# artis-mcrt/artis

Hardware: AMD Instinct MI355X
Metric: packet-steps/sec (higher is better)
Workload: dtype f64

## Files before the change

### artis_amd/csrc/artis_engine.hip

```cpp
#include <hip/hip_runtime.h>
#include <rccl/rccl.h>

#include <dlfcn.h>

#include <cstdio>
#include <cstdlib>
#include <algorithm>
#include <chrono>
#include <cstring>
#include <string>
#include <type_traits>
#include <utility>
#include <vector>
#include <cmath>

#include "model_build.h"
#include "engine_config.h"
#include "physics.h"
#include "radfield_fit.h"
#include "ion_balance.h"
#include "spectra.h"

#include <rocprim/device/device_radix_sort.hpp>

// ... 821 lines not shown
        kind = NEXT_RPKT;
      } else {
        kind = kpkt_blackbody_case(env, type, cellindex) ? NEXT_BB : NEXT_KPKT;
      }
    }
  }
  append_by_kind(kind, (int32_t)i, cellindex, nu_cmf, L);
}

__global__ void __launch_bounds__(BLOCK) k_count_waiting(Env env, int32_t *counts, int32_t *other) {
  const int64_t i = (int64_t)blockIdx.x * BLOCK + threadIdx.x;
  if (i >= env.P.n) return;
  const PktHot &h = env.P.hot[i];
  const int type = h.type;
  const bool active = type_handled(type) && h.prop_time < env.S.ts_end;
  const bool waiting = h.pend != PEND_NONE || h.ma_level >= 0;
  if (!(waiting || active)) return;
  const int c = env.M.propcell_nonemptymgi[h.cellindex];
  if ((active && type_gamma(type) && !waiting) || c < 0)
    atomicAdd(other, 1);
  else
    atomicAdd(&counts[c], 1);
}
__global__ void __launch_bounds__(BLOCK) k_sort_hist(const int32_t *keys, int32_t n, int32_t *hist) {
  const int64_t i = (int64_t)blockIdx.x * BLOCK + threadIdx.x;
  if (i < n) atomicAdd(&hist[keys[i]], 1);
}
constexpr int SCAN_TILE = 8192;
__global__ void __launch_bounds__(1024) k_scan_tiles(int32_t *hist, int32_t nkeys, int32_t *tile_totals) {
  __shared__ int32_t part[1024];
  const int t = threadIdx.x;
  const int64_t base = (int64_t)blockIdx.x * SCAN_TILE + (int64_t)t * 8;
  int32_t v[8];
  int32_t sum = 0;
#pragma unroll
  for (int k = 0; k < 8; k++) {
    v[k] = (base + k < nkeys) ? hist[base + k] : 0;
    sum += v[k];
  }
  part[t] = sum;
  __syncthreads();
  for (int off = 1; off < 1024; off <<= 1) {
    const int32_t add = (t >= off) ? part[t - off] : 0;
    __syncthreads();
    part[t] += add;
    __syncthreads();
  }
  int32_t run = part[t] - sum;
#pragma unroll
// ... 9 lines not shown
  int32_t carry = 0;
  for (int start = 0; start < ntiles; start += 1024) {
    const int i = start + t;
    const int32_t v = (i < ntiles) ? tile_totals[i] : 0;
    part[t] = v;
    __syncthreads();
    for (int off = 1; off < 1024; off <<= 1) {
      const int32_t add = (t >= off) ? part[t - off] : 0;
      __syncthreads();
      part[t] += add;
      __syncthreads();
    }
    if (i < ntiles) tile_totals[i] = carry + part[t] - v;
    carry += part[1023];
    __syncthreads();
  }
}
__global__ void __launch_bounds__(1024) k_scan_add(int32_t *hist, int32_t nkeys, const int32_t *tile_totals) {
  const int32_t off = tile_totals[blockIdx.x];
  const int64_t base = (int64_t)blockIdx.x * SCAN_TILE + (int64_t)threadIdx.x * 8;
#pragma unroll
  for (int k = 0; k < 8; k++)
    if (base + k < nkeys) hist[base + k] += off;
}
__global__ void __launch_bounds__(BLOCK) k_sort_scatter(const int32_t *list, const int32_t *keys, int32_t n, int32_t *offsets, int32_t *out) {
  const int64_t i = (int64_t)blockIdx.x * BLOCK + threadIdx.x;
  if (i < n) out[atomicAdd(&offsets[keys[i]], 1)] = list[i];
}
constexpr int SORT_LDS_KEYS = 8192;
constexpr int SORT_LDS_GRID = 2048;
__global__ void __launch_bounds__(BLOCK) k_sort_hist_lds(const int32_t *keys, int32_t n, int32_t *hist, int32_t nkeys) {
  __shared__ int32_t h[SORT_LDS_KEYS];
  for (int k = threadIdx.x; k < nkeys; k += BLOCK) h[k] = 0;
  __syncthreads();
  const int64_t chunk = ((int64_t)n + gridDim.x - 1) / gridDim.x;
  const int64_t lo = chunk * blockIdx.x, hi = (lo + chunk < n) ? lo + chunk : n;
  for (int64_t i = lo + threadIdx.x; i < hi; i += BLOCK) atomicAdd(&h[keys[i]], 1);
  __syncthreads();
  for (int k = threadIdx.x; k < nkeys; k += BLOCK)
    if (h[k] != 0) atomicAdd(&hist[k], h[k]);
}
__global__ void __launch_bounds__(BLOCK) k_sort_scatter_lds(const int32_t *list, const int32_t *keys, int32_t n, int32_t *offsets, int32_t *out,
                                                            int32_t nkeys) {
  __shared__ int32_t h[SORT_LDS_KEYS];
  for (int k = threadIdx.x; k < nkeys; k += BLOCK) h[k] = 0;
  __syncthreads();
  const int64_t chunk = ((int64_t)n + gridDim.x - 1) / gridDim.x;
  const int64_t lo = chunk * blockIdx.x, hi = (lo + chunk < n) ? lo + chunk : n;
  for (int64_t i = lo + threadIdx.x; i < hi; i += BLOCK) atomicAdd(&h[keys[i]], 1);
  __syncthreads();
// ... 1139 lines not shown
  }
  __syncthreads();
  if (threadIdx.x < ARTIS_NSTATS && lstats[threadIdx.x] != 0) atomicAdd(&gstats[threadIdx.x], lstats[threadIdx.x]);
}
#endif

inline int nblocks(int64_t n) { return (int)((n + BLOCK - 1) / BLOCK); }

struct SpecState;
void spec_free(SpecState *st);
struct RfState;
void rf_free(RfState *st);
struct IbState;
void ib_free(IbState *st);

}

struct LastCall {
  double propagate_ms = 0., kms[NEXT_NKINDS] = {}, kms_tail = 0., fill_ms = 0.;
  int64_t klaunches[NEXT_NKINDS] = {}, kthreads[NEXT_NKINDS] = {}, nlaunches = 0;
  int64_t sweeps = 0, tile_fills = 0, sparse_fills = 0, cells_filled = 0, listed = 0, parked = 0;
  int64_t pool_resets = 0;
  int32_t thermal_variants = 0, est_forms = 0;
};
struct artis_amd_engine {
  int device = 0;
  EngineConfig cfg;
  double cache_budget = 0.;
  SpecState *spec = nullptr;
  RfState *rf = nullptr;
  IbState *ib = nullptr;
  bool fit_since_step = false;
  ModelOwned own;
  std::vector<void *> model_allocs;
  std::vector<void *> cell_allocs;
  std::vector<void *> cache_allocs;
  DevModel M{};
  DevModel Mh{};
  artis_model model_copy{};
  std::vector<int32_t> own_matransblock_start;
  DevCells C{};
  DevCache K{};
  DevStep S{};
  DevEst E{};
  bool have_cells = false;
  bool expopac_own = false;
// ... 21 lines not shown
  int32_t *d_target_level = nullptr;
  double *d_est = nullptr;
  int64_t est_ndoubles = 0;
  int64_t nvspec = 0, nvgrid = 0;
  unsigned long long *d_stats = nullptr;
  int32_t *d_err = nullptr;
  int32_t *h_counts = nullptr;
  int64_t npackets = -1;
  void *d_pkt = nullptr;
  void *d_pkt_snapshot = nullptr;
  size_t pkt_bytes = 0;
  PktStore P{};
  artis_packet *d_aos = nullptr;
  int64_t aos_capacity = 0;
  bool aos_valid = false;
  int32_t *d_lists[NEXT_NKINDS][2] = {};
  int32_t *d_keys[NEXT_NKINDS][2] = {};
  int32_t *d_sorted = nullptr;
  int32_t *d_perm = nullptr;
  bool use_perm = false;
  bool slot_order_by_cell = true;
  int32_t *d_hist = nullptr;
  int32_t *d_tiles = nullptr;
  int32_t *d_count = nullptr;
  int32_t *d_cursors = nullptr;
  int ncu = 256;
  double *d_gamma_ws = nullptr;
  int32_t *d_gamma_gi = nullptr;
  int32_t *d_gamma_n = nullptr;
  int64_t ws_capacity = 0;
  hipEvent_t ev0 = nullptr, ev1 = nullptr, ev2 = nullptr, ev3 = nullptr;
  LastCall last;
  int tail_max = ARTIS_OPT_DETAILED_BF_ESTIMATORS_ON ? 16384 : 4096;
  bool tail_always = false;
  int32_t *d_fill_cells = nullptr;
  bool sparse_fill = true;
  int64_t sparse_max_listed = 16384;
  bool park_tails = true;
  int64_t park_at = 3145728;
  int64_t last_pool_used = 0, last_pool_cap = 0;
  double ma_hotfrac = 1.;
  bool vpkt_cont_lds = true;
  bool tile_zigzag = false;
  bool tile_adapt = true;
  int64_t tile_block = 0;
  bool pool_keep = true;
// ... 157 lines not shown
  env.S = e->S;
  env.E = e->E;
  env.est_stride = 8;
  env.pair_stride = 2;
  env.P = e->P;
  env.stats = nullptr;
  env.gamma_ws = e->d_gamma_ws;
  env.bfev = e->bf_defer ? e->d_bfev : nullptr;
  env.bfev_count = e->d_bfev_count;
  env.bfev_cap = e->bfev_cap;
  env.bfrate_kept = (e->bf_defer && e->ntiles == 1) ? e->d_bfrate_kept : nullptr;
  env.gamma_gi = e->d_gamma_gi;
  env.gamma_n = e->d_gamma_n;
  env.errflag = e->d_err;
  env.vpkt_queue = e->d_vpkt_queue;
  env.vpkt_count = e->d_vpkt_count;
  env.vpkt_cap = e->vpkt_cap;
#ifdef ARTIS_VISIT_COUNTS
  env.visit_counts = e->d_visit_counts;
#endif
  return env;
}

void free_packet_buffers(artis_amd_engine *e) {
  void **singles[] = {&e->d_pkt, &e->d_pkt_snapshot, (void **)&e->d_sorted, (void **)&e->d_perm, (void **)&e->d_gamma_ws,
                      (void **)&e->d_gamma_gi, (void **)&e->d_gamma_n, (void **)&e->d_bfev, (void **)&e->d_bfev_count,
                      (void **)&e->d_vpkt_queue, (void **)&e->d_vpkt_count};
  e->bfev_cap = 0;
  e->vpkt_cap = 0;
  for (void **q : singles) {
    if (*q) (void)hipFree(*q);
    *q = nullptr;
  }
  for (int kind = 0; kind < NEXT_NKINDS; kind++)
    for (int k = 0; k < 2; k++) {
      if (e->d_lists[kind][k]) (void)hipFree(e->d_lists[kind][k]);
      if (e->d_keys[kind][k]) (void)hipFree(e->d_keys[kind][k]);
      e->d_lists[kind][k] = nullptr;
      e->d_keys[kind][k] = nullptr;
    }
  e->npackets = -1;
  e->use_perm = false;
}

int ensure_packet_buffers(artis_amd_engine *e, int64_t n) {
  if (n == e->npackets && e->d_pkt) return ARTIS_OK;
  free_packet_buffers(e);
  e->pkt_bytes = pkt_store_bytes(n);
  HIP_TRY(hipMalloc(&e->d_pkt, e->pkt_bytes));
  e->P = carve_pkt_store(e->d_pkt, n);
  const size_t listbytes = sizeof(int32_t) * (size_t)(n > 0 ? n : 1);
  for (int kind = 1; kind < NEXT_NKINDS; kind++)
    for (int k = 0; k < 2; k++) {
      HIP_TRY(hipMalloc((void **)&e->d_lists[kind][k], listbytes));
      HIP_TRY(hipMalloc((void **)&e->d_keys[kind][k], listbytes));
    }
  HIP_TRY(hipMalloc((void **)&e->d_sorted, listbytes));
  HIP_TRY(hipMalloc((void **)&e->d_perm, listbytes));
  e->ws_capacity = n > 0 ? n : 1;
  const size_t wsbytes = sizeof(double) * (size_t)(e->Mh.nbfcontinua_ground + 1) * (size_t)e->ws_capacity;
  HIP_TRY(hipMalloc((void **)&e->d_gamma_ws, wsbytes));
  HIP_TRY(hipMalloc((void **)&e->d_gamma_gi, wsbytes / 2));
  HIP_TRY(hipMalloc((void **)&e->d_gamma_n, sizeof(int32_t) * (size_t)e->ws_capacity));
  HIP_TRY(hipMemset(e->d_gamma_n, 0, sizeof(int32_t) * (size_t)e->ws_capacity));
#if ARTIS_OPT_DETAILED_BF_ESTIMATORS_ON
  if (e->Mh.nbfcontinua > 0) {
    const int64_t cap = std::min<int64_t>((int64_t)(n > 0 ? n : 1) * e->budget_r, 0x7FFFFFF0LL);
    HIP_TRY(hipMalloc((void **)&e->d_bfev, sizeof(BfEvent) * (size_t)cap));
    HIP_TRY(hipMalloc((void **)&e->d_bfev_count, sizeof(int32_t)));
    HIP_TRY(hipMemset(e->d_bfev_count, 0, sizeof(int32_t)));
    e->bfev_cap = (int32_t)cap;
  }
#endif
#if ARTIS_OPT_VPKT_ON
  {
    const int64_t cap = std::min<int64_t>((int64_t)(n > 0 ? n : 1) * std::max(e->budget_r, 1), 0x7FFFFFF0LL);
    HIP_TRY(hipMalloc((void **)&e->d_vpkt_queue, sizeof(VpktSeed) * (size_t)cap));
    HIP_TRY(hipMalloc((void **)&e->d_vpkt_count, sizeof(int32_t)));
    HIP_TRY(hipMemset(e->d_vpkt_count, 0, sizeof(int32_t)));
    e->vpkt_cap = (int32_t)cap;
  }
// ... 265 lines not shown
        return ARTIS_ERR_ARG;
      }
    }
  {
    int64_t next = 0;
    for (int ul = 0; ul < model->nlevels; ul++) {
      if (model->level_alltrans_startdown[ul] != next || model->level_ndowntrans[ul] < 0 || model->level_nuptrans[ul] < 0) {
        g_last_error = "alltrans is not contiguous in level order (level_alltrans_startdown[i+1] == startdown[i] + ndown[i] + nup[i])";
        return ARTIS_ERR_ARG;
      }
      next += (int64_t)model->level_ndowntrans[ul] + model->level_nuptrans[ul];
    }
    if (next != model->nalltrans) {
      g_last_error = "the last level's transitions do not end at nalltrans";
      return ARTIS_ERR_ARG;
    }
  }
  for (int i = 0; i < model->nions; i++) {
    if (model->ion_nlevels[i] > 65535) {
      g_last_error = "an ion has more levels than a 16-bit target level can describe";
      return ARTIS_ERR_UNSUPPORTED;
    }
  }
  return ARTIS_OK;
}
}

extern "C" {

size_t artis_amd_sizeof_config(void) { return sizeof(artis_amd_config); }
size_t artis_amd_sizeof_plan(void) { return sizeof(artis_amd_plan); }
void artis_amd_config_default(artis_amd_config *cfg) {
  if (cfg) config_set_default(cfg);
}

int artis_amd_engine_create(const artis_model *model, int device, artis_amd_engine **out) {
  return artis_amd_engine_create_ex(model, device, nullptr, out);
}

int artis_amd_engine_create_ex(const artis_model *model, int device, const artis_amd_config *cfg, artis_amd_engine **out) {
  if (out) *out = nullptr;
  if (!model || !out) {
    g_last_error = "null argument";
    return ARTIS_ERR_ARG;
  }
  artis_amd_config checked;
// ... 176 lines not shown
  HIP_TRY(hipMalloc((void **)&e->d_stats, sizeof(unsigned long long) * ARTIS_NSTATS));
  HIP_TRY(hipMemset(e->d_stats, 0, sizeof(unsigned long long) * ARTIS_NSTATS));
  HIP_TRY(hipMalloc((void **)&e->d_count, sizeof(int32_t) * (2 * NEXT_NKINDS + 1)));
  HIP_TRY(hipMemset(e->d_count, 0, sizeof(int32_t) * (2 * NEXT_NKINDS + 1)));
  e->d_err = e->d_count + (2 * NEXT_NKINDS);
  HIP_TRY(hipHostMalloc((void **)&e->h_counts, sizeof(int32_t) * (2 * NEXT_NKINDS + 1), hipHostMallocDefault));
  HIP_TRY(hipMalloc((void **)&e->d_cursors, sizeof(int32_t) * (MAX_CHUNKS + 1)));
  HIP_TRY(hipMalloc((void **)&e->d_fill_cells, sizeof(int32_t) * (size_t)(ncell_all > 0 ? ncell_all : 1)));
  if (e->ntiles > 1) {
    HIP_TRY(hipMalloc((void **)&e->d_krow, sizeof(int32_t) * (size_t)ncell_all));
    e->h_krow.assign((size_t)ncell_all, -1);
    e->h_wanted.assign((size_t)ncell_all, 0);
    e->h_rowcell.assign((size_t)e->tile_cells, -1);
    HIP_TRY(hipMemset(e->d_krow, 0xFF, sizeof(int32_t) * (size_t)ncell_all));
    e->h_cell_grid.assign((size_t)ncell_all, 0);
    for (int g = 0; g < h.ngrid; g++)
      if (h.propcell_nonemptymgi[g] >= 0) e->h_cell_grid[(size_t)h.propcell_nonemptymgi[g]] = g;
  }
  {
    hipDeviceProp_t prop;
    HIP_TRY(hipGetDeviceProperties(&prop, device));
    e->ncu = prop.multiProcessorCount > 0 ? prop.multiProcessorCount : 256;
  }
  HIP_TRY(hipMalloc((void **)&e->d_hist, sizeof(int32_t) * ((size_t)h.ngrid * SORT_NUBINS + 1)));
  HIP_TRY(hipMalloc((void **)&e->d_tiles, sizeof(int32_t) * (((size_t)h.ngrid * SORT_NUBINS) / SCAN_TILE + 2)));
  HIP_TRY(hipEventCreate(&e->ev0));
  HIP_TRY(hipEventCreate(&e->ev1));
  HIP_TRY(hipEventCreate(&e->ev2));
  HIP_TRY(hipEventCreate(&e->ev3));
  read_switches(e);
  {
    const int64_t nrows_ = e->tile_cells;
    Env env0 = make_env(e);
    env0.K = e->K;
    hipLaunchKernelGGL(k_mainit, dim3(nblocks(nrows_ * e->Mh.nlevels)), dim3(BLOCK), 0, nullptr, env0, nrows_);
    HIP_TRY(hipGetLastError());
    HIP_TRY(hipDeviceSynchronize());
  }
  {
    e->pop_batch = pop_batch_cells(e->Mh, e->tile_cells, e->cfg);
    HIP_TRY(hipMalloc((void **)&e->d_collexc_terms, pop_scratch_alloc_bytes(e->Mh, e->pop_batch)));
  }
  if (e->trace) trace_config(e);
  if (e->trace)
    fprintf(stderr, "[artis_amd] record tiers: static records for %.2f of every ion's levels, %d cold levels, pool of %d slots per resident cell; %d tile(s) of %lld cells, %zu B per cell\n",
            e->ma_hotfrac, e->Mh.ncold, e->Mh.ma_pool_slots, e->ntiles, (long long)e->tile_cells, e->cache_bytes_per_cell);
  return ARTIS_OK;
}
// ... 434 lines not shown

int artis_amd_packets_upload(artis_amd_engine *e, const artis_packet *packets, int64_t npackets) {
  if (!e || (!packets && npackets > 0) || npackets < 0 || npackets > 2147483000LL) {
    g_last_error = "bad packet buffer";
    return ARTIS_ERR_ARG;
  }
  HIP_TRY(hipSetDevice(e->device));
  int rc = ensure_packet_buffers(e, npackets);
  if (rc != ARTIS_OK) return rc;
  rc = ensure_aos(e, npackets);
  if (rc != ARTIS_OK) return rc;
  if (e->d_pkt_snapshot) (void)hipFree(e->d_pkt_snapshot);
  e->d_pkt_snapshot = nullptr;
  if (npackets > 0) {
    HIP_TRY(hipMemcpy(e->d_aos, packets, sizeof(artis_packet) * (size_t)npackets, hipMemcpyHostToDevice));
    e->aos_valid = true;
    e->use_perm = false;
    if (e->slot_order_by_cell && e->sort_lists && npackets >= 2 * BLOCK) {
      int32_t *ident = e->d_lists[NEXT_RPKT][0], *keys = e->d_lists[NEXT_RPKT][1];
      const int32_t n32 = (int32_t)npackets;
      const int32_t nkeys = e->Mh.ngrid;
      hipStream_t s = nullptr;
      hipLaunchKernelGGL(k_aos_cellkeys, dim3(nblocks(npackets)), dim3(BLOCK), 0, s, e->d_aos, npackets, nkeys, ident, keys);
      HIP_TRY(hipMemsetAsync(e->d_hist, 0, sizeof(int32_t) * (size_t)(nkeys + 1), s));
      if (nkeys <= SORT_LDS_KEYS)
        hipLaunchKernelGGL(k_sort_hist_lds, dim3(sort_lds_grid(n32)), dim3(BLOCK), 0, s, keys, n32, e->d_hist, nkeys);
      else
        hipLaunchKernelGGL(k_sort_hist, dim3(nblocks(n32)), dim3(BLOCK), 0, s, keys, n32, e->d_hist);
      const int ntiles = (nkeys + SCAN_TILE - 1) / SCAN_TILE;
      hipLaunchKernelGGL(k_scan_tiles, dim3(ntiles), dim3(1024), 0, s, e->d_hist, nkeys, e->d_tiles);
      hipLaunchKernelGGL(k_scan_totals, dim3(1), dim3(1024), 0, s, e->d_tiles, ntiles);
      hipLaunchKernelGGL(k_scan_add, dim3(ntiles), dim3(1024), 0, s, e->d_hist, nkeys, e->d_tiles);
      if (nkeys <= SORT_LDS_KEYS)
        hipLaunchKernelGGL(k_sort_scatter_lds, dim3(sort_lds_grid(n32)), dim3(BLOCK), 0, s, ident, keys, n32, e->d_hist, e->d_perm, nkeys);
      else
        hipLaunchKernelGGL(k_sort_scatter, dim3(nblocks(n32)), dim3(BLOCK), 0, s, ident, keys, n32, e->d_hist, e->d_perm);
      e->use_perm = true;
    }
    hipLaunchKernelGGL(k_aos_to_rec, dim3(nblocks(npackets)), dim3(BLOCK), 0, nullptr, e->d_aos, e->P, e->use_perm ? e->d_perm : nullptr);
    HIP_TRY(hipGetLastError());
    HIP_TRY(hipDeviceSynchronize());
  }
  return ARTIS_OK;
}

int artis_amd_packets_download(artis_amd_engine *e, artis_packet *packets, int64_t npackets) {
  if (!e || npackets != e->npackets || (!packets && npackets > 0)) {
    g_last_error = "packet count does not match the resident population";
    return ARTIS_ERR_ARG;
  }
  HIP_TRY(hipSetDevice(e->device));
  if (npackets == 0) return ARTIS_OK;
  int rc = ensure_aos(e, npackets);
  if (rc != ARTIS_OK) return rc;
  if (!e->aos_valid) HIP_TRY(hipMemcpy(e->d_aos, packets, sizeof(artis_packet) * (size_t)npackets, hipMemcpyHostToDevice));
  hipLaunchKernelGGL(k_rec_to_aos, dim3(nblocks(npackets)), dim3(BLOCK), 0, nullptr, e->P, e->d_aos, e->use_perm ? e->d_perm : nullptr);
  HIP_TRY(hipGetLastError());
  HIP_TRY(hipMemcpy(packets, e->d_aos, sizeof(artis_packet) * (size_t)npackets, hipMemcpyDeviceToHost));
  return ARTIS_OK;
// ... 322 lines not shown
    if (matrans) HIP_TRY(hipMemcpy(matrans, d_trans, sizeof(double) * (size_t)h.nmatransblock, hipMemcpyDeviceToHost));
    (void)hipFree(d_rates);
    (void)hipFree(d_trans);
    (void)hipFree(d_bad);
    if (bad != 0) {
      g_last_error = std::to_string(bad) + " filter entries of the cell's macro-atom records differ from the sequential form";
      return ARTIS_ERR_NOTCONVERGED;
    }
  }
  DL(allcont_nnlevel, allcont_nnlevel, double, h.nbfcontinua)
  DL(allcont_departure, allcont_departure, double, h.nbfcontinua)
  DL(allcont_edgepart, allcont_edgepart, double, h.nbfcontinua)
  if (allcont_keepbits && h.nbfcontinua > 0)
    HIP_TRY(hipMemcpy(allcont_keepbits, e->K.allcont_keepbits + (int64_t)c * h.nkeepwords, sizeof(uint64_t) * (size_t)((h.nbfcontinua + 63) / 64),
                      hipMemcpyDeviceToHost));
  DL(corrphotoioncoeff, corrphotoioncoeff, double, h.nphixstargets_total)
  DL(cooling_contrib, cooling_contrib, double, h.ncoolingterms)
  DL(ion_cooling_contribs, ion_cooling_contribs, double, h.nions)
  DL(chi_ff_nnionpart, chi_ff_nnionpart, double, 1)
#undef DL
  return ARTIS_OK;
}

}

#include "stage_propagate.h"
#include "stage_common.h"
#include "stage_spectra.h"
#include "stage_radfield.h"
#include "stage_ionbal.h"
```

### artis_amd/csrc/stage_propagate.h

```cpp
#pragma once
namespace {
#define STEP(expr)                     \
  do {                                 \
    const int _rc = (expr);            \
    if (_rc != ARTIS_OK) return _rc;   \
  } while (0)
template <int N>
using Int = std::integral_constant<int, N>;
int sort_by_key(artis_amd_engine *e, hipStream_t s, const int32_t *list, const int32_t *keys, int32_t n, const int32_t **out, int nbins,
                int64_t ncells, int max_per_cell, int32_t nkeys_given = 0) {
  *out = list;
  if (!e->sort_lists || n < 2 * BLOCK) return ARTIS_OK;
  if ((int64_t)n > (int64_t)max_per_cell * (ncells > 0 ? ncells : 1)) return ARTIS_OK;
  const int32_t nkeys = nkeys_given > 0 ? nkeys_given : e->Mh.ngrid * nbins;
  HIP_TRY(hipMemsetAsync(e->d_hist, 0, sizeof(int32_t) * (size_t)(nkeys + 1), s));
  if (nkeys <= SORT_LDS_KEYS)
    hipLaunchKernelGGL(k_sort_hist_lds, dim3(sort_lds_grid(n)), dim3(BLOCK), 0, s, keys, n, e->d_hist, nkeys);
  else
    hipLaunchKernelGGL(k_sort_hist, dim3(nblocks(n)), dim3(BLOCK), 0, s, keys, n, e->d_hist);
  const int ntiles = (nkeys + SCAN_TILE - 1) / SCAN_TILE;
  hipLaunchKernelGGL(k_scan_tiles, dim3(ntiles), dim3(1024), 0, s, e->d_hist, nkeys, e->d_tiles);
  hipLaunchKernelGGL(k_scan_totals, dim3(1), dim3(1024), 0, s, e->d_tiles, ntiles);
  hipLaunchKernelGGL(k_scan_add, dim3(ntiles), dim3(1024), 0, s, e->d_hist, nkeys, e->d_tiles);
  if (nkeys <= SORT_LDS_KEYS)
    hipLaunchKernelGGL(k_sort_scatter_lds, dim3(sort_lds_grid(n)), dim3(BLOCK), 0, s, list, keys, n, e->d_hist, e->d_sorted, nkeys);
  else
    hipLaunchKernelGGL(k_sort_scatter, dim3(nblocks(n)), dim3(BLOCK), 0, s, list, keys, n, e->d_hist, e->d_sorted);
  *out = e->d_sorted;
  return ARTIS_OK;
}
#if ARTIS_OPT_DETAILED_BF_ESTIMATORS_ON
void launch_bfest_dense(artis_amd_engine *e, const Env &env, hipStream_t s) {
  const bool lds = e->dense_cont_lds && e->Mh.nbfcontinua <= CONT_LDS_MAX;
  e->last.est_forms |= (lds ? ARTIS_AMD_EST_BF_DENSE_CONTLDS : ARTIS_AMD_EST_BF_DENSE_HBM) |
                       (e->dense_lpr == 64 ? ARTIS_AMD_EST_BF_LPR64 : (e->dense_lpr == 16 ? ARTIS_AMD_EST_BF_LPR16 : ARTIS_AMD_EST_BF_LPR32));
  auto launch = [&](auto lpr) {
    if (lds)
      hipLaunchKernelGGL((k_bfest_dense<true, DENSE_TB, decltype(lpr)::value>), dim3(e->ncu * ARTIS_DENSE_WGS), dim3(DENSE_TB), 0, s, env);
    else
      hipLaunchKernelGGL((k_bfest_dense<false, BLOCK, decltype(lpr)::value>), dim3(e->ncu * 8), dim3(BLOCK), 0, s, env);
  };
  if (e->dense_lpr == 64)
    launch(Int<64>{});
  else if (e->dense_lpr == 16)
    launch(Int<16>{});
  else
    launch(Int<32>{});
}
#endif
std::string errflag_text(int32_t flag, bool at_call_end) {
// ... 394 lines not shown
```

### artis_amd/engine.py

```python
from __future__ import annotations

import ctypes as C
import os

import numpy as np

from . import abi
from .build import SO, build, so_path


class EngineError(RuntimeError):
    pass


_LIBS = {}


def load_library(build_if_missing: bool = False, preset: str = "classic"):
    if preset in _LIBS:
        return _LIBS[preset]
    so = so_path(preset)
    so = os.environ.get("ARTIS_AMD_SO" if preset == "classic" else f"ARTIS_AMD_SO_{preset.upper()}", so)
    if not os.path.exists(so):
        if not build_if_missing:
# ... 27 lines not shown
    L.artis_amd_last_kernel_ms.argtypes = [C.c_void_p, C.POINTER(C.c_double), C.POINTER(C.c_int64)]
    L.artis_amd_spectra_compute.argtypes = [C.c_void_p, C.POINTER(abi.SpectraConfig), C.c_void_p]
    L.artis_amd_spectra_devptr.argtypes = [C.c_void_p, C.POINTER(C.c_void_p), C.POINTER(C.c_int64)]
    L.artis_amd_spectra_download.argtypes = [C.c_void_p, C.POINTER(abi.Spectra)]
    L.artis_amd_radfield_fit.argtypes = [C.c_void_p, C.POINTER(abi.RadfieldConfig), C.c_void_p]
    L.artis_amd_radfield_download.argtypes = [C.c_void_p, C.POINTER(abi.Radfield)]
    L.artis_amd_grid_update.argtypes = [C.c_void_p, C.POINTER(abi.GridUpdate), C.c_void_p, C.c_void_p]
    L.artis_amd_grid_update_download.argtypes = [C.c_void_p, C.POINTER(abi.GridUpdateResult)]
    if L.artis_amd_abi_version() != abi.ABI_VERSION:
        raise EngineError(f"{so}: ABI version {L.artis_amd_abi_version()}, this package describes version {abi.ABI_VERSION}")
    assert L.artis_amd_sizeof_packet() == abi.PACKET_DTYPE.itemsize
    assert L.artis_amd_sizeof_config() == C.sizeof(abi.Config) and L.artis_amd_sizeof_plan() == C.sizeof(abi.Plan)
    L.artis_amd_options_preset.restype = C.c_char_p
    assert L.artis_amd_options_preset().decode() == preset, (L.artis_amd_options_preset(), preset)
    _LIBS[preset] = L
    return L


EXPORTED_SYMBOLS = [
    "artis_amd_last_error", "artis_amd_abi_version", "artis_amd_sizeof_packet", "artis_amd_engine_create",
    "artis_amd_engine_destroy", "artis_amd_set_cellstate", "artis_amd_update_packets", "artis_amd_packets_upload",
    "artis_amd_packets_download", "artis_amd_packets_snapshot", "artis_amd_packets_restore",
    "artis_amd_update_packets_device", "artis_amd_estimators_zero", "artis_amd_estimators_download",
    "artis_amd_estimators_devptr", "artis_amd_last_kernel_ms", "artis_amd_debug_cellcache", "artis_amd_debug_visit_counts", "artis_amd_last_kernel_ms_by_kind",
    "artis_amd_populate_cellcache",
    "artis_amd_last_kernel_breakdown",
    "artis_amd_last_kernel_launches",
    "artis_amd_last_kernel_table",
    "artis_amd_options_preset",
    "artis_amd_allreduce_estimators", "artis_amd_comm_unique_id", "artis_amd_comm_init", "artis_amd_comm_count",
    "artis_amd_cache_tiles", "artis_amd_last_tiling", "artis_amd_last_tiling_fills", "artis_amd_last_tiling_parked", "artis_amd_last_pool_resets", "artis_amd_record_tiers", "artis_amd_last_thermal_variants", "artis_amd_last_estimator_forms", "artis_amd_last_pool_usage",
    "artis_amd_spectra_compute", "artis_amd_spectra_devptr", "artis_amd_spectra_download",
    "artis_amd_radfield_fit", "artis_amd_radfield_download",
    "artis_amd_grid_update", "artis_amd_grid_update_download",
    "artis_amd_sizeof_config", "artis_amd_config_default", "artis_amd_engine_create_ex", "artis_amd_engine_config",
    "artis_amd_sizeof_plan", "artis_amd_engine_plan",
]


def _as_config(config) -> abi.Config:
    return config if isinstance(config, abi.Config) else abi.config(**config)


def plan(model: abi.Model, config=None, device: int = 0, preset: str = "classic", free_bytes: int = 0) -> dict:
    L = load_library(preset=preset)
    out = abi.Plan(struct_size=C.sizeof(abi.Plan))
    cfg = C.byref(_as_config(config)) if config is not None else None
# ... 161 lines not shown
        out["uppermost_ion"] = out["uppermost_ion"].reshape(n, ne)
        out["gamma_normed"] = out["gamma_normed"][: n * g].reshape(n, g)
        out["ncells_flagged"] = {k: int(info.ncells_flagged[i]) for i, k in enumerate(abi.IONBAL_FLAGS)}
        out["total_evals"] = int(info.total_evals)
        out["kernel_ms"] = tuple(float(x) for x in info.kernel_ms)
        return out

    def debug_cellcache(self, c: int) -> dict:
        d = self.model.d
        out = {
            "levelpops": np.zeros(d["nlevels"]), "maprocessrates": np.zeros(d["nlevels"] * 9),
            "matrans": np.zeros(max(d["nmatransblock"], 1)), "allcont_nnlevel": np.zeros(max(d["nbfcontinua"], 1)),
            "allcont_departure": np.zeros(max(d["nbfcontinua"], 1)), "allcont_edgepart": np.zeros(max(d["nbfcontinua"], 1)),
            "allcont_keepbits": np.zeros((d["nbfcontinua"] + 63) // 64 + 1, dtype=np.uint64),
            "corrphotoioncoeff": np.zeros(max(d["nphixstargets_total"], 1)),
            "cooling_contrib": np.zeros(max(d["ncoolingterms"], 1)), "ion_cooling_contribs": np.zeros(d["nions"]),
        }
        chi = C.c_double(0.0)
        args = [self.h, C.c_int(c)] + [v.ctypes.data_as(C.c_void_p) for v in out.values()] + [C.byref(chi)]
        self._check(self.L.artis_amd_debug_cellcache(*args))
        out["chi_ff_nnionpart"] = chi.value
        return out

    def config(self) -> dict:
        out = abi.config()
        self._check(self.L.artis_amd_engine_config(self.h, C.byref(out)))
        return abi.struct_dict(out)

    def cache_tiles(self):
        nt, cells, bpc = C.c_int32(), C.c_int64(), C.c_int64()
        self.L.artis_amd_cache_tiles.argtypes = [C.c_void_p] * 4
        self._check(self.L.artis_amd_cache_tiles(self.h, C.byref(nt), C.byref(cells), C.byref(bpc)))
        return nt.value, cells.value, bpc.value

    def record_tiers(self):
        h, n, p = C.c_double(), C.c_int32(), C.c_int64()
        self.L.artis_amd_record_tiers.argtypes = [C.c_void_p] * 4
        self._check(self.L.artis_amd_record_tiers(self.h, C.byref(h), C.byref(n), C.byref(p)))
        return {"hot_fraction": h.value, "ncold": n.value, "pool_slots": p.value}

    THERMAL_PLAIN, THERMAL_LDS_TABLES, THERMAL_LDS_LEVELPACK, THERMAL_REFILL, THERMAL_COLD, THERMAL_TAIL = 1, 2, 4, 8, 16, 32

    def last_thermal_variants(self) -> int:
        m = C.c_int32()
        self.L.artis_amd_last_thermal_variants.argtypes = [C.c_void_p] * 2
        self._check(self.L.artis_amd_last_thermal_variants(self.h, C.byref(m)))
# ... 79 lines not shown
```

### include/artis_amd.h

```cpp
#ifndef ARTIS_AMD_H
#define ARTIS_AMD_H

#include <stddef.h>
#include <stdint.h>

#ifdef __cplusplus
extern "C" {
#endif

enum {
  ARTIS_TYPE_NONE = 0,
  ARTIS_TYPE_GAMMA = 10,
  ARTIS_TYPE_RPKT = 11,
  ARTIS_TYPE_KPKT = 12,
  ARTIS_TYPE_MA = 13,
  ARTIS_TYPE_NTLEPTON_DEPOSITED = 20,
  ARTIS_TYPE_NONTHERMAL_PREDEPOSIT_BETAMINUS = 21,
  ARTIS_TYPE_NONTHERMAL_PREDEPOSIT_BETAPLUS = 22,
  ARTIS_TYPE_NONTHERMAL_PREDEPOSIT_ALPHA = 23,
  ARTIS_TYPE_NTALPHA_FISPROD_DEPOSITED = 24,
  ARTIS_TYPE_ESCAPE = 32,
  ARTIS_TYPE_RADIOACTIVE_PELLET = 100,
  ARTIS_TYPE_PRE_KPKT = 120
};
// ... 420 lines not shown
#define ARTIS_AMD_EST_THERMAL_LDS 16
#define ARTIS_AMD_EST_THERMAL_WAVECACHE 32
#define ARTIS_AMD_EST_THERMAL_GLOBAL 64
#define ARTIS_AMD_EST_GAMMA_LDS 128
#define ARTIS_AMD_EST_GAMMA_GLOBAL 256
#define ARTIS_AMD_EST_BF_INPLACE 512
#define ARTIS_AMD_EST_BF_DENSE_CONTLDS 1024
#define ARTIS_AMD_EST_BF_DENSE_HBM 2048
#define ARTIS_AMD_EST_BF_LPR16 4096
#define ARTIS_AMD_EST_BF_LPR32 8192
#define ARTIS_AMD_EST_BF_LPR64 16384
int artis_amd_last_estimator_forms(artis_amd_engine *eng, int32_t *mask);

int artis_amd_last_kernel_breakdown(artis_amd_engine *eng, double *rpkt_ms, int64_t *rpkt_threads, double *thermal_ms,
                                    int64_t *thermal_threads);

int artis_amd_last_kernel_launches(artis_amd_engine *eng, int64_t *rpkt_launches, int64_t *thermal_launches);
int artis_amd_last_kernel_table(artis_amd_engine *eng, double ms[4], int64_t launches[4], int64_t packets[4]);

int artis_amd_debug_cellcache(artis_amd_engine *eng, int nonemptymgi, double *levelpops, double *maprocessrates,
                              double *matrans, double *allcont_nnlevel, double *allcont_departure,
                              double *allcont_edgepart, uint64_t *allcont_keepbits, double *corrphotoioncoeff,
                              double *cooling_contrib, double *ion_cooling_contribs, double *chi_ff_nnionpart);

int artis_amd_last_kernel_ms_by_kind(artis_amd_engine *eng, double ms[8], int64_t launches[8]);

int artis_amd_debug_visit_counts(artis_amd_engine *eng, uint32_t *counts, int64_t n);

#define ARTIS_SPEC_MNUBINS 1000
#define ARTIS_SPEC_MABINS 100
#define ARTIS_SPEC_ALL_DIRBINS (-2)
typedef struct artis_spectra_config {
  int64_t struct_size;
  int32_t ntimesteps;
  int32_t dirbin;
  const double *ts_start;
  const double *ts_width;
  double tmin, tmax;
  int32_t emission_absorption;
  int32_t stokes;
  int32_t gamma;
  int32_t reserved;
} artis_spectra_config;
typedef struct artis_spectra {
  int64_t struct_size;
  double *lum, *lumcmf, *flux, *flux_q, *flux_u, *emission, *emission_q, *emission_u, *trueemission, *absorption, *absorption_q,
// ... 91 lines not shown
```

Measured before the change: 1.376 billion.

## Replace global-atomic counting sort with two-pass tiled radix sort for many keys

For work lists whose key space exceeds the LDS histogram limit, the sort changes from a global-atomic histogram and scatter over the whole key range to a two-level scheme. The first level buckets by the high key bits using per-tile LDS histograms, a scanned tile matrix and a stable scatter into key/value pairs. The second level sorts each bucket by its low bits in LDS-sized chunks. This removes contended global atomics and the large memset and scan over ngrid*nbins histogram entries, at the cost of more kernel launches and a pair buffer. It also caps the supported key count and adds a debug entry point.

```diff
diff --git a/artis_amd/csrc/artis_engine.hip b/artis_amd/csrc/artis_engine.hip
--- a/artis_amd/csrc/artis_engine.hip
+++ b/artis_amd/csrc/artis_engine.hip
@@ -867,9 +867,125 @@
   else
     atomicAdd(&counts[c], 1);
 }
-__global__ void __launch_bounds__(BLOCK) k_sort_hist(const int32_t *keys, int32_t n, int32_t *hist) {
-  const int64_t i = (int64_t)blockIdx.x * BLOCK + threadIdx.x;
-  if (i < n) atomicAdd(&hist[keys[i]], 1);
+constexpr int SORT_HI_BITS = 11;
+constexpr int SORT_HI_MAX = 1 << SORT_HI_BITS;
+constexpr int SORT_LO_BITS_MAX = 14;
+constexpr int64_t SORT_MAX_KEYS = (int64_t)1 << (SORT_HI_BITS + SORT_LO_BITS_MAX);
+constexpr int SORT_TILE = 8192;
+constexpr int SORT_TB = 512;
+constexpr int SORT_SEG_CAP = 8192;
+__global__ void __launch_bounds__(SORT_TB) k_sort_tilehist(const int32_t *keys, int32_t n, int lobits, int nb, int32_t ntiles, int32_t *mat) {
+  __shared__ int32_t h[SORT_HI_MAX];
+  for (int b = threadIdx.x; b < nb; b += SORT_TB) h[b] = 0;
+  __syncthreads();
+  const int64_t lo = (int64_t)blockIdx.x * SORT_TILE, hi = (lo + SORT_TILE < n) ? lo + SORT_TILE : n;
+  for (int64_t i = lo + threadIdx.x; i < hi; i += SORT_TB) atomicAdd(&h[keys[i] >> lobits], 1);
+  __syncthreads();
+  for (int b = threadIdx.x; b < nb; b += SORT_TB) mat[(int64_t)b * ntiles + blockIdx.x] = h[b];
+}
+__global__ void __launch_bounds__(SORT_TB) k_sort_tilescatter(const int32_t *list, const int32_t *keys, int32_t n, int lobits, int nb, int32_t ntiles,
+                                                              const int32_t *mat, int2 *pairs) {
+  __shared__ int32_t h[SORT_HI_MAX];
+  for (int b = threadIdx.x; b < nb; b += SORT_TB) h[b] = mat[(int64_t)b * ntiles + blockIdx.x];
+  __syncthreads();
+  const int64_t lo = (int64_t)blockIdx.x * SORT_TILE, hi = (lo + SORT_TILE < n) ? lo + SORT_TILE : n;
+  for (int64_t i = lo + threadIdx.x; i < hi; i += SORT_TB) {
+    const int32_t k = keys[i];
+    pairs[atomicAdd(&h[k >> lobits], 1)] = make_int2(k, list[i]);
+  }
+}
+__global__ void __launch_bounds__(1024) k_sort_plan(const int32_t *mat, int32_t ntiles, int nb, int32_t n, int32_t *seg, int32_t *chunk_base) {
+  __shared__ int32_t part[1024];
+  const int t = threadIdx.x;
+  int32_t c[2];
+#pragma unroll
+  for (int k = 0; k < 2; k++) {
+    const int b = 2 * t + k;
+    c[k] = 0;
+    if (b < nb) {
+      const int32_t s0 = mat[(int64_t)b * ntiles], s1 = (b + 1 < nb) ? mat[(int64_t)(b + 1) * ntiles] : n;
+      seg[b] = s0;
+      c[k] = (s1 - s0 + SORT_SEG_CAP - 1) / SORT_SEG_CAP;
+    }
+  }
+  if (t == 0) seg[nb] = n;
+  part[t] = c[0] + c[1];
+  __syncthreads();
+  for (int off = 1; off < 1024; off <<= 1) {
+    const int32_t add = (t >= off) ? part[t - off] : 0;
+    __syncthreads();
+    part[t] += add;
+    __syncthreads();
+  }
+  const int32_t run = part[t] - c[0] - c[1];
+  if (2 * t < nb) chunk_base[2 * t] = run;
+  if (2 * t + 1 < nb) chunk_base[2 * t + 1] = run + c[0];
+  if (t == 1023) chunk_base[nb] = part[1023];
+}
+__global__ void __launch_bounds__(BLOCK) k_sort_segments(const int2 *pairs, int lobits, int nb, const int32_t *seg, const int32_t *chunk_base,
+                                                         int32_t *out) {
+  extern __shared__ int32_t sm[];
+  __shared__ int32_t part[BLOCK];
+  __shared__ int s_bucket;
+  const int t = threadIdx.x;
+  const int nlow = 1 << lobits, mask = nlow - 1;
+  if (t == 0) {
+    int b = -1;
+    if ((int32_t)blockIdx.x < chunk_base[nb]) {
+      int lo = 0, hi = nb - 1;
+      while (lo < hi) {
+        const int mid = (lo + hi + 1) >> 1;
+        if (chunk_base[mid] <= (int32_t)blockIdx.x)
+          lo = mid;
+        else
+          hi = mid - 1;
+      }
+      b = lo;
+    }
+    s_bucket = b;
+  }
+  __syncthreads();
+  const int b = s_bucket;
+  if (b < 0) return;
+  const int32_t s0 = seg[b], s1 = seg[b + 1];
+  const int32_t c0 = s0 + ((int32_t)blockIdx.x - chunk_base[b]) * SORT_SEG_CAP, c1 = (s1 - c0 > SORT_SEG_CAP) ? c0 + SORT_SEG_CAP : s1;
+  int32_t *tot = sm, *before = sm + nlow;
+  const bool later = c0 > s0;
+  for (int d = t; d < nlow; d += BLOCK) {
+    tot[d] = 0;
+    if (later) before[d] = 0;
+  }
+  __syncthreads();
+  for (int32_t i = s0 + t; i < c0; i += BLOCK) {
+    const int d = pairs[i].x & mask;
+    atomicAdd(&tot[d], 1);
+    atomicAdd(&before[d], 1);
+  }
+  for (int32_t i = c0 + t; i < s1; i += BLOCK) atomicAdd(&tot[pairs[i].x & mask], 1);
+  __syncthreads();
+  const int per = (nlow + BLOCK - 1) / BLOCK;
+  const int d0 = (t * per < nlow) ? t * per : nlow, d1 = (d0 + per < nlow) ? d0 + per : nlow;
+  int32_t sum = 0;
+  for (int d = d0; d < d1; d++) sum += tot[d];
+  part[t] = sum;
+  __syncthreads();
+  for (int off = 1; off < BLOCK; off <<= 1) {
+    const int32_t add = (t >= off) ? part[t - off] : 0;
+    __syncthreads();
+    part[t] += add;
+    __syncthreads();
+  }
+  int32_t run = part[t] - sum;
+  for (int d = d0; d < d1; d++) {
+    const int32_t v = tot[d];
+    tot[d] = run + (later ? before[d] : 0);
+    run += v;
+  }
+  __syncthreads();
+  for (int32_t i = c0 + t; i < c1; i += BLOCK) {
+    const int2 p = pairs[i];
+    out[s0 + atomicAdd(&tot[p.x & mask], 1)] = p.y;
+  }
 }
 constexpr int SCAN_TILE = 8192;
 __global__ void __launch_bounds__(1024) k_scan_tiles(int32_t *hist, int32_t nkeys, int32_t *tile_totals) {
@@ -925,10 +1041,6 @@
 #pragma unroll
   for (int k = 0; k < 8; k++)
     if (base + k < nkeys) hist[base + k] += off;
-}
-__global__ void __launch_bounds__(BLOCK) k_sort_scatter(const int32_t *list, const int32_t *keys, int32_t n, int32_t *offsets, int32_t *out) {
-  const int64_t i = (int64_t)blockIdx.x * BLOCK + threadIdx.x;
-  if (i < n) out[atomicAdd(&offsets[keys[i]], 1)] = list[i];
 }
 constexpr int SORT_LDS_KEYS = 8192;
 constexpr int SORT_LDS_GRID = 2048;
@@ -2114,6 +2226,15 @@
   int64_t sweeps = 0, tile_fills = 0, sparse_fills = 0, cells_filled = 0, listed = 0, parked = 0;
   int64_t pool_resets = 0;
   int32_t thermal_variants = 0, est_forms = 0;
+};
+struct SortScratch {
+  void *base = nullptr;
+  int64_t capacity = 0;
+  int2 *pairs = nullptr;
+  int32_t *mat = nullptr;
+  int32_t *tiles = nullptr;
+  int32_t *seg = nullptr;
+  int32_t *chunk_base = nullptr;
 };
 struct artis_amd_engine {
   int device = 0;
@@ -2181,6 +2302,8 @@
   bool slot_order_by_cell = true;
   int32_t *d_hist = nullptr;
   int32_t *d_tiles = nullptr;
+  SortScratch sort_scratch;
+  bool sort_attr_set = false;
   int32_t *d_count = nullptr;
   int32_t *d_cursors = nullptr;
   int ncu = 256;
@@ -2384,12 +2507,84 @@
   return env;
 }
 
+void sort_scratch_free(SortScratch &S) {
+  if (S.base) (void)hipFree(S.base);
+  S = SortScratch{};
+}
+int sort_scratch_alloc(SortScratch &S, int64_t n) {
+  sort_scratch_free(S);
+  const size_t cap = (size_t)(n > 0 ? n : 1);
+  const size_t matlen = (size_t)SORT_HI_MAX * ((cap + SORT_TILE - 1) / SORT_TILE);
+  auto padded = [](size_t bytes) { return (bytes + 255) & ~(size_t)255; };
+  const size_t b_pairs = padded(sizeof(int2) * cap), b_mat = padded(sizeof(int32_t) * matlen), b_tiles = padded(sizeof(int32_t) * (matlen / SCAN_TILE + 2)),
+               b_seg = padded(sizeof(int32_t) * (SORT_HI_MAX + 1));
+  HIP_TRY(hipMalloc(&S.base, b_pairs + b_mat + b_tiles + 2 * b_seg));
+  char *q = (char *)S.base;
+  S.pairs = (int2 *)q;
+  S.mat = (int32_t *)(q += b_pairs);
+  S.tiles = (int32_t *)(q += b_mat);
+  S.seg = (int32_t *)(q += b_tiles);
+  S.chunk_base = (int32_t *)(q += b_seg);
+  S.capacity = (int64_t)cap;
+  return ARTIS_OK;
+}
+std::string sort_too_many_keys_text(int64_t nkeys) {
+  return "the work-list sort takes at most " + std::to_string(SORT_MAX_KEYS) + " keys (cells x bins), this list has " + std::to_string(nkeys) +
+         ": run without sorted lists (ARTIS_AMD_SORT=0)";
+}
+int sort_many_keys(artis_amd_engine *e, const SortScratch &S, hipStream_t s, const int32_t *list, const int32_t *keys, int32_t n, int64_t nkeys,
+                   int32_t *out) {
+  if (nkeys > SORT_MAX_KEYS) {
+    g_last_error = sort_too_many_keys_text(nkeys);
+    return ARTIS_ERR_UNSUPPORTED;
+  }
+  if (n <= 0 || n > S.capacity) {
+    g_last_error = "sort: the list does not fit the sort's buffers";
+    return ARTIS_ERR_ARG;
+  }
+  int keybits = 0;
+  while (((int64_t)1 << keybits) < nkeys) keybits++;
+  const int lobits = std::max(0, keybits - SORT_HI_BITS);
+  const int nb = (int)((nkeys - 1) >> lobits) + 1;
+  const int32_t ntiles = (int32_t)(((int64_t)n + SORT_TILE - 1) / SORT_TILE);
+  const int32_t matlen = nb * ntiles;
+  const int nscan = (matlen + SCAN_TILE - 1) / SCAN_TILE;
+  const size_t lds = sizeof(int32_t) * 2 * ((size_t)1 << lobits);
+  if (lds > 32 * 1024 && !e->sort_attr_set) {
+    HIP_TRY(hipFuncSetAttribute((const void *)k_sort_segments, hipFuncAttributeMaxDynamicSharedMemorySize, (int)(sizeof(int32_t) * 2 << SORT_LO_BITS_MAX)));
+    e->sort_attr_set = true;
+  }
+  hipLaunchKernelGGL(k_sort_tilehist, dim3(ntiles), dim3(SORT_TB), 0, s, keys, n, lobits, nb, ntiles, S.mat);
+  hipLaunchKernelGGL(k_scan_tiles, dim3(nscan), dim3(1024), 0, s, S.mat, matlen, S.tiles);
+  if (nscan > 1) {
+    hipLaunchKernelGGL(k_scan_totals, dim3(1), dim3(1024), 0, s, S.tiles, nscan);
+    hipLaunchKernelGGL(k_scan_add, dim3(nscan), dim3(1024), 0, s, S.mat, matlen, S.tiles);
+  }
+  hipLaunchKernelGGL(k_sort_tilescatter, dim3(ntiles), dim3(SORT_TB), 0, s, list, keys, n, lobits, nb, ntiles, S.mat, S.pairs);
+  hipLaunchKernelGGL(k_sort_plan, dim3(1), dim3(1024), 0, s, S.mat, ntiles, nb, n, S.seg, S.chunk_base);
+  hipLaunchKernelGGL(k_sort_segments, dim3(n / SORT_SEG_CAP + nb), dim3(BLOCK), lds, s, S.pairs, lobits, nb, S.seg, S.chunk_base, out);
+  return ARTIS_OK;
+}
+int sort_list(artis_amd_engine *e, hipStream_t s, const int32_t *list, const int32_t *keys, int32_t n, int64_t nkeys, int32_t *out) {
+  if (nkeys > SORT_LDS_KEYS) return sort_many_keys(e, e->sort_scratch, s, list, keys, n, nkeys, out);
+  const int32_t nk = (int32_t)nkeys;
+  HIP_TRY(hipMemsetAsync(e->d_hist, 0, sizeof(int32_t) * (size_t)(nk + 1), s));
+  hipLaunchKernelGGL(k_sort_hist_lds, dim3(sort_lds_grid(n)), dim3(BLOCK), 0, s, keys, n, e->d_hist, nk);
+  const int ntiles = (nk + SCAN_TILE - 1) / SCAN_TILE;
+  hipLaunchKernelGGL(k_scan_tiles, dim3(ntiles), dim3(1024), 0, s, e->d_hist, nk, e->d_tiles);
+  hipLaunchKernelGGL(k_scan_totals, dim3(1), dim3(1024), 0, s, e->d_tiles, ntiles);
+  hipLaunchKernelGGL(k_scan_add, dim3(ntiles), dim3(1024), 0, s, e->d_hist, nk, e->d_tiles);
+  hipLaunchKernelGGL(k_sort_scatter_lds, dim3(sort_lds_grid(n)), dim3(BLOCK), 0, s, list, keys, n, e->d_hist, out, nk);
+  return ARTIS_OK;
+}
+
 void free_packet_buffers(artis_amd_engine *e) {
   void **singles[] = {&e->d_pkt, &e->d_pkt_snapshot, (void **)&e->d_sorted, (void **)&e->d_perm, (void **)&e->d_gamma_ws,
                       (void **)&e->d_gamma_gi, (void **)&e->d_gamma_n, (void **)&e->d_bfev, (void **)&e->d_bfev_count,
                       (void **)&e->d_vpkt_queue, (void **)&e->d_vpkt_count};
   e->bfev_cap = 0;
   e->vpkt_cap = 0;
+  sort_scratch_free(e->sort_scratch);
   for (void **q : singles) {
     if (*q) (void)hipFree(*q);
     *q = nullptr;
@@ -2419,6 +2614,7 @@
     }
   HIP_TRY(hipMalloc((void **)&e->d_sorted, listbytes));
   HIP_TRY(hipMalloc((void **)&e->d_perm, listbytes));
+  if (const int rc = sort_scratch_alloc(e->sort_scratch, n)) return rc;
   e->ws_capacity = n > 0 ? n : 1;
   const size_t wsbytes = sizeof(double) * (size_t)(e->Mh.nbfcontinua_ground + 1) * (size_t)e->ws_capacity;
   HIP_TRY(hipMalloc((void **)&e->d_gamma_ws, wsbytes));
@@ -2730,6 +2926,14 @@
       return ARTIS_ERR_UNSUPPORTED;
     }
   }
+  {
+    const char *b = std::getenv("ARTIS_AMD_SORT");
+    const int64_t nkeys = (int64_t)model->ngrid * SORT_NUBINS;
+    if (nkeys > SORT_MAX_KEYS && !(b && std::atoi(b) == 0)) {
+      g_last_error = sort_too_many_keys_text(nkeys);
+      return ARTIS_ERR_UNSUPPORTED;
+    }
+  }
   return ARTIS_OK;
 }
 }
@@ -2952,8 +3156,8 @@
     HIP_TRY(hipGetDeviceProperties(&prop, device));
     e->ncu = prop.multiProcessorCount > 0 ? prop.multiProcessorCount : 256;
   }
-  HIP_TRY(hipMalloc((void **)&e->d_hist, sizeof(int32_t) * ((size_t)h.ngrid * SORT_NUBINS + 1)));
-  HIP_TRY(hipMalloc((void **)&e->d_tiles, sizeof(int32_t) * (((size_t)h.ngrid * SORT_NUBINS) / SCAN_TILE + 2)));
+  HIP_TRY(hipMalloc((void **)&e->d_hist, sizeof(int32_t) * (SORT_LDS_KEYS + 1)));
+  HIP_TRY(hipMalloc((void **)&e->d_tiles, sizeof(int32_t) * (SORT_LDS_KEYS / SCAN_TILE + 2)));
   HIP_TRY(hipEventCreate(&e->ev0));
   HIP_TRY(hipEventCreate(&e->ev1));
   HIP_TRY(hipEventCreate(&e->ev2));
@@ -3434,19 +3638,7 @@
       const int32_t nkeys = e->Mh.ngrid;
       hipStream_t s = nullptr;
       hipLaunchKernelGGL(k_aos_cellkeys, dim3(nblocks(npackets)), dim3(BLOCK), 0, s, e->d_aos, npackets, nkeys, ident, keys);
-      HIP_TRY(hipMemsetAsync(e->d_hist, 0, sizeof(int32_t) * (size_t)(nkeys + 1), s));
-      if (nkeys <= SORT_LDS_KEYS)
-        hipLaunchKernelGGL(k_sort_hist_lds, dim3(sort_lds_grid(n32)), dim3(BLOCK), 0, s, keys, n32, e->d_hist, nkeys);
-      else
-        hipLaunchKernelGGL(k_sort_hist, dim3(nblocks(n32)), dim3(BLOCK), 0, s, keys, n32, e->d_hist);
-      const int ntiles = (nkeys + SCAN_TILE - 1) / SCAN_TILE;
-      hipLaunchKernelGGL(k_scan_tiles, dim3(ntiles), dim3(1024), 0, s, e->d_hist, nkeys, e->d_tiles);
-      hipLaunchKernelGGL(k_scan_totals, dim3(1), dim3(1024), 0, s, e->d_tiles, ntiles);
-      hipLaunchKernelGGL(k_scan_add, dim3(ntiles), dim3(1024), 0, s, e->d_hist, nkeys, e->d_tiles);
-      if (nkeys <= SORT_LDS_KEYS)
-        hipLaunchKernelGGL(k_sort_scatter_lds, dim3(sort_lds_grid(n32)), dim3(BLOCK), 0, s, ident, keys, n32, e->d_hist, e->d_perm, nkeys);
-      else
-        hipLaunchKernelGGL(k_sort_scatter, dim3(nblocks(n32)), dim3(BLOCK), 0, s, ident, keys, n32, e->d_hist, e->d_perm);
+      if (const int rc2 = sort_list(e, s, ident, keys, n32, nkeys, e->d_perm)) return rc2;
       e->use_perm = true;
     }
     hipLaunchKernelGGL(k_aos_to_rec, dim3(nblocks(npackets)), dim3(BLOCK), 0, nullptr, e->d_aos, e->P, e->use_perm ? e->d_perm : nullptr);
@@ -3815,6 +4007,55 @@
   return ARTIS_OK;
 }
 
+
+int artis_amd_debug_sort_list(artis_amd_engine *e, const int32_t *keys, const int32_t *list, int32_t n, int64_t nkeys, int32_t *out) {
+  if (!e || n < 0 || (n > 0 && (!keys || !list || !out))) {
+    g_last_error = "null argument or negative length";
+    return ARTIS_ERR_ARG;
+  }
+  if (nkeys <= SORT_LDS_KEYS) {
+    g_last_error = "debug_sort_list runs the many-keys sort: nkeys has to be above " + std::to_string(SORT_LDS_KEYS);
+    return ARTIS_ERR_ARG;
+  }
+  if (nkeys > SORT_MAX_KEYS) {
+    g_last_error = sort_too_many_keys_text(nkeys);
+    return ARTIS_ERR_UNSUPPORTED;
+  }
+  for (int32_t i = 0; i < n; i++)
+    if (keys[i] < 0 || keys[i] >= nkeys) {
+      g_last_error = "a key is outside [0, nkeys)";
+      return ARTIS_ERR_ARG;
+    }
+  if (n < 2 * BLOCK) {
+    if (n > 0) std::memcpy(out, list, sizeof(int32_t) * (size_t)n);
+    return ARTIS_OK;
+  }
+  HIP_TRY(hipSetDevice(e->device));
+  SortScratch &S = e->sort_scratch;
+  int32_t *d_io = nullptr;
+  int rc = (S.capacity >= n) ? ARTIS_OK : sort_scratch_alloc(S, n);
+  if (rc == ARTIS_OK && hipMalloc((void **)&d_io, sizeof(int32_t) * 3 * (size_t)n) != hipSuccess) {
+    g_last_error = "debug_sort_list: out of device memory";
+    rc = ARTIS_ERR_HIP;
+  }
+  auto copy = [&](void *dst, const void *src, hipMemcpyKind kind) {
+    if (rc == ARTIS_OK && hipMemcpy(dst, src, sizeof(int32_t) * (size_t)n, kind) != hipSuccess) {
+      g_last_error = "debug_sort_list: copy failed";
+      rc = ARTIS_ERR_HIP;
+    }
+  };
+  copy(d_io, keys, hipMemcpyHostToDevice);
+  copy(d_io + n, list, hipMemcpyHostToDevice);
+  if (rc == ARTIS_OK) rc = sort_many_keys(e, S, nullptr, d_io + n, d_io, n, nkeys, d_io + 2 * (size_t)n);
+  if (rc == ARTIS_OK && (hipGetLastError() != hipSuccess || hipDeviceSynchronize() != hipSuccess)) {
+    g_last_error = "debug_sort_list: a sort kernel failed";
+    rc = ARTIS_ERR_HIP;
+  }
+  copy(out, d_io + 2 * (size_t)n, hipMemcpyDeviceToHost);
+  if (d_io) (void)hipFree(d_io);
+  return rc;
+}
+
 }
 
 #include "stage_propagate.h"
diff --git a/artis_amd/csrc/stage_propagate.h b/artis_amd/csrc/stage_propagate.h
--- a/artis_amd/csrc/stage_propagate.h
+++ b/artis_amd/csrc/stage_propagate.h
@@ -12,20 +12,7 @@
   *out = list;
   if (!e->sort_lists || n < 2 * BLOCK) return ARTIS_OK;
   if ((int64_t)n > (int64_t)max_per_cell * (ncells > 0 ? ncells : 1)) return ARTIS_OK;
-  const int32_t nkeys = nkeys_given > 0 ? nkeys_given : e->Mh.ngrid * nbins;
-  HIP_TRY(hipMemsetAsync(e->d_hist, 0, sizeof(int32_t) * (size_t)(nkeys + 1), s));
-  if (nkeys <= SORT_LDS_KEYS)
-    hipLaunchKernelGGL(k_sort_hist_lds, dim3(sort_lds_grid(n)), dim3(BLOCK), 0, s, keys, n, e->d_hist, nkeys);
-  else
-    hipLaunchKernelGGL(k_sort_hist, dim3(nblocks(n)), dim3(BLOCK), 0, s, keys, n, e->d_hist);
-  const int ntiles = (nkeys + SCAN_TILE - 1) / SCAN_TILE;
-  hipLaunchKernelGGL(k_scan_tiles, dim3(ntiles), dim3(1024), 0, s, e->d_hist, nkeys, e->d_tiles);
-  hipLaunchKernelGGL(k_scan_totals, dim3(1), dim3(1024), 0, s, e->d_tiles, ntiles);
-  hipLaunchKernelGGL(k_scan_add, dim3(ntiles), dim3(1024), 0, s, e->d_hist, nkeys, e->d_tiles);
-  if (nkeys <= SORT_LDS_KEYS)
-    hipLaunchKernelGGL(k_sort_scatter_lds, dim3(sort_lds_grid(n)), dim3(BLOCK), 0, s, list, keys, n, e->d_hist, e->d_sorted, nkeys);
-  else
-    hipLaunchKernelGGL(k_sort_scatter, dim3(nblocks(n)), dim3(BLOCK), 0, s, list, keys, n, e->d_hist, e->d_sorted);
+  STEP(sort_list(e, s, list, keys, n, nkeys_given > 0 ? (int64_t)nkeys_given : (int64_t)e->Mh.ngrid * nbins, e->d_sorted));
   *out = e->d_sorted;
   return ARTIS_OK;
 }
diff --git a/artis_amd/engine.py b/artis_amd/engine.py
--- a/artis_amd/engine.py
+++ b/artis_amd/engine.py
@@ -73,7 +73,7 @@
     "artis_amd_engine_destroy", "artis_amd_set_cellstate", "artis_amd_update_packets", "artis_amd_packets_upload",
     "artis_amd_packets_download", "artis_amd_packets_snapshot", "artis_amd_packets_restore",
     "artis_amd_update_packets_device", "artis_amd_estimators_zero", "artis_amd_estimators_download",
-    "artis_amd_estimators_devptr", "artis_amd_last_kernel_ms", "artis_amd_debug_cellcache", "artis_amd_debug_visit_counts", "artis_amd_last_kernel_ms_by_kind",
+    "artis_amd_estimators_devptr", "artis_amd_last_kernel_ms", "artis_amd_debug_cellcache", "artis_amd_debug_sort_list", "artis_amd_debug_visit_counts", "artis_amd_last_kernel_ms_by_kind",
     "artis_amd_populate_cellcache",
     "artis_amd_last_kernel_breakdown",
     "artis_amd_last_kernel_launches",
@@ -281,6 +281,16 @@
         out["chi_ff_nnionpart"] = chi.value
         return out
 
+    def debug_sort_list(self, keys, lst, nkeys: int):
+        keys = np.ascontiguousarray(keys, dtype=np.int32)
+        lst = np.ascontiguousarray(lst, dtype=np.int32)
+        assert keys.shape == lst.shape and keys.ndim == 1
+        out = np.empty_like(lst)
+        self.L.artis_amd_debug_sort_list.argtypes = [C.c_void_p, C.c_void_p, C.c_void_p, C.c_int32, C.c_int64, C.c_void_p]
+        self._check(self.L.artis_amd_debug_sort_list(self.h, keys.ctypes.data_as(C.c_void_p), lst.ctypes.data_as(C.c_void_p), len(lst), int(nkeys),
+                                                     out.ctypes.data_as(C.c_void_p)))
+        return out
+
     def config(self) -> dict:
         out = abi.config()
         self._check(self.L.artis_amd_engine_config(self.h, C.byref(out)))
diff --git a/include/artis_amd.h b/include/artis_amd.h
--- a/include/artis_amd.h
+++ b/include/artis_amd.h
@@ -466,6 +466,7 @@
                               double *matrans, double *allcont_nnlevel, double *allcont_departure,
                               double *allcont_edgepart, uint64_t *allcont_keepbits, double *corrphotoioncoeff,
                               double *cooling_contrib, double *ion_cooling_contribs, double *chi_ff_nnionpart);
+int artis_amd_debug_sort_list(artis_amd_engine *eng, const int32_t *keys, const int32_t *list, int32_t n, int64_t nkeys, int32_t *out);
 
 int artis_amd_last_kernel_ms_by_kind(artis_amd_engine *eng, double ms[8], int64_t launches[8]);
 
```

Result: faster. 1.420 billion, median of 6 (+3.2%).
